# scwolof/gp_grief

Hardware: AMD Instinct MI355X
Metric: CG iters/sec + Kron-matvec achieved HBM GB/s, 4D RBF grid 200^4 (higher is better)
Workload: dtype f64

## Files before the change

### gp_grief_amd/csrc/gg_kronb.hip

```cpp
#include <algorithm>
#include <cmath>
#include <cstdlib>
#include <vector>

#include "gg_internal.h"

namespace gg {

typedef double bd4 __attribute__((ext_vector_type(4)));

constexpr int kBlkMaxD = 6;
constexpr int kBlkModeWaves = 12;
constexpr int kBlkPairWaves = 4;

struct BlockOp {
  int d = 0;
  int64_t m[kBlkMaxD] = {}, h[kBlkMaxD] = {};
  int64_t e[kBlkMaxD] = {};
  int64_t nb = 0, n = 0;
  double* frag[kBlkMaxD][2] = {};
  int KS[kBlkMaxD] = {}, JT[kBlkMaxD] = {};
  bool T4[kBlkMaxD] = {};
  int pTF = 0;
  int cus = 256;
  bool pair_lds = false;
  int pair_spw = 1;
  bool fast = true;
  bool pro_nt = true;
  bool epi_nt = true;
};

struct FoldGeom {
  int d;
  int64_t m[kBlkMaxD], h[kBlkMaxD], stride[kBlkMaxD];
  int64_t hp;
  int64_t nb;
  int64_t blk0, nblk;
};

template <int D>
__global__ __launch_bounds__(256) void blk_fold_kernel(const double* __restrict__ x,
                                                       double* __restrict__ y, FoldGeom g,
                                                       int inverse, double scale,
                                                       double* __restrict__ sq_part) {
  constexpr int C = 1 << D;
  double acc = 0.0;
  for (int64_t t = (int64_t)blockIdx.x * blockDim.x + threadIdx.x; t < g.nb;
       t += (int64_t)gridDim.x * blockDim.x) {
    int64_t lo = 0, span[D];
    const int64_t hs = g.hp;
    const int64_t q = t % (hs * hs);
    int64_t rem = t / (hs * hs);
    {
      const int64_t a4 = q / (4 * hs), r4 = q - a4 * 4 * hs;
      const int64_t i = r4 >> 2, a = 4 * a4 + (r4 & 3);
      if (i >= g.h[D - 2] || a >= g.h[D - 1]) {
        if (!inverse)
          for (int c = 0; c < C; ++c) {
            const int64_t lb = (int64_t)c - g.blk0;
            if (lb >= 0 && lb < g.nblk) y[lb * g.nb + t] = 0.0;
          }
        continue;
      }
      lo = i * g.stride[D - 2] + a * g.stride[D - 1];
      span[D - 2] = (g.m[D - 2] - 1 - 2 * i) * g.stride[D - 2];
      span[D - 1] = (g.m[D - 1] - 1 - 2 * a) * g.stride[D - 1];
    }
#pragma unroll
    for (int k = D - 3; k >= 0; --k) {
      const int64_t i = rem % g.h[k];
      rem /= g.h[k];
      lo += i * g.stride[k];
      span[k] = (g.m[k] - 1 - 2 * i) * g.stride[k];
    }
    double v[C];
    if (!inverse) {
#pragma unroll
      for (int c = 0; c < C; ++c) {
        int64_t o = lo;
#pragma unroll
        for (int k = 0; k < D; ++k)
          if ((c >> (D - 1 - k)) & 1) o += span[k];
        v[c] = x[o];
      }
    } else {
#pragma unroll
      for (int c = 0; c < C; ++c) {
        const int64_t lb = (int64_t)c - g.blk0;
        v[c] = (lb >= 0 && lb < g.nblk) ? x[lb * g.nb + t] : 0.0;
      }
    }
#pragma unroll
    for (int b = 1; b < C; b <<= 1)
#pragma unroll
      for (int c = 0; c < C; ++c)
        if (!(c & b)) {
          const double a0 = v[c], a1 = v[c | b];
          v[c] = a0 + a1;
          v[c | b] = a0 - a1;
        }
    if (!inverse) {
#pragma unroll
      for (int c = 0; c < C; ++c) {
        const int64_t lb = (int64_t)c - g.blk0;
        if (lb < 0 || lb >= g.nblk) continue;
        const double w = v[c] * scale;
        y[lb * g.nb + t] = w;
        acc = fma(w, w, acc);
      }
    } else {
#pragma unroll
      for (int c = 0; c < C; ++c) {
        int64_t o = lo;
#pragma unroll
        for (int k = 0; k < D; ++k)
          if ((c >> (D - 1 - k)) & 1) o += span[k];
        y[o] = v[c] * scale;
      }
    }
  }
  if (sq_part != nullptr) {
#pragma unroll
    for (int off = 32; off > 0; off >>= 1) acc += __shfl_xor(acc, off, 64);
    __shared__ double red[4];
    if ((threadIdx.x & 63) == 0) red[threadIdx.x >> 6] = acc;
    __syncthreads();
    if (threadIdx.x == 0) sq_part[blockIdx.x] = red[0] + red[1] + red[2] + red[3];
  }
}

__device__ __forceinline__ char* ubase(const void* p, int64_t off) {
  const uint64_t v = reinterpret_cast<uint64_t>(p) + (uint64_t)off;
  const uint32_t lo = __builtin_amdgcn_readfirstlane((uint32_t)v);
  const uint32_t hi = __builtin_amdgcn_readfirstlane((uint32_t)(v >> 32));
  uint64_t u = ((uint64_t)hi << 32) | lo;
  asm("" : "+s"(u));
  return reinterpret_cast<char*>(u);
}
__device__ __forceinline__ int64_t uni64(int64_t x) {
  const uint32_t lo = __builtin_amdgcn_readfirstlane((uint32_t)x);
  const uint32_t hi = __builtin_amdgcn_readfirstlane((uint32_t)((uint64_t)x >> 32));
  return (int64_t)(((uint64_t)hi << 32) | lo);
}
typedef __attribute__((address_space(1))) char gchar;
typedef __attribute__((address_space(1))) double gdouble;
__device__ __forceinline__ double ldu(const void* p, int64_t uoff, uint32_t voff) {
  gchar* b = reinterpret_cast<gchar*>(reinterpret_cast<uintptr_t>(ubase(p, uoff)));
  return *reinterpret_cast<const gdouble*>(b + voff);
}
__device__ __forceinline__ void stu(void* p, int64_t uoff, uint32_t voff, double v) {
  gchar* b = reinterpret_cast<gchar*>(reinterpret_cast<uintptr_t>(ubase(p, uoff)));
  *reinterpret_cast<gdouble*>(b + voff) = v;
}
template <bool NT>
__device__ __forceinline__ double lduq(const void* p, int64_t uoff, uint32_t voff) {
  if constexpr (!NT) return ldu(p, uoff, voff);
  gchar* b = reinterpret_cast<gchar*>(reinterpret_cast<uintptr_t>(ubase(p, uoff)));
  return __builtin_nontemporal_load(reinterpret_cast<const gdouble*>(b + voff));
}
template <bool NT>
__device__ __forceinline__ void stuq(void* p, int64_t uoff, uint32_t voff, double v) {
  if constexpr (!NT) {
    stu(p, uoff, voff, v);
  } else {
    gchar* b = reinterpret_cast<gchar*>(reinterpret_cast<uintptr_t>(ubase(p, uoff)));
    __builtin_nontemporal_store(v, reinterpret_cast<gdouble*>(b + voff));
  }
}
typedef double gd2v __attribute__((ext_vector_type(2)));
typedef __attribute__((address_space(1))) gd2v gd2;
__device__ __forceinline__ double2 ld2g(const double* p) {
  const gd2v v = *reinterpret_cast<const gd2*>(reinterpret_cast<uintptr_t>(p));
  return double2{v.x, v.y};
}
__device__ __forceinline__ void st2g(double* p, double2 v) {
  *reinterpret_cast<gd2*>(reinterpret_cast<uintptr_t>(p)) = gd2v{v.x, v.y};
}
struct ModeArgs {
  const double* X;
  double* Y;
  const double* fS;
  const double* fT;
  int h, KS;
  int64_t inner;
  int64_t spb;
  int64_t gpb;
  int64_t ngroups;
  int64_t per_wg;
  int64_t nb;
  int bitpos;
  int64_t blk0;
  const int* skip;
  double* r;
  const double* q_old;
  double* p_out;
  const CgScalars* sc;
  double* rr_part;
  int64_t pqo_stride;
  const double* pprev;
  const double* coef;
  double* sx;
  int64_t soff, sn, soff_h1, sn_h1, sstep;
};

template <int JT, bool T4, int KIND>
__global__ __launch_bounds__(64 * kBlkModeWaves, 1) void blk_mode_kernel(ModeArgs a) {
  constexpr int W = kBlkModeWaves;
  constexpr int TF = T4 ? JT - 1 : JT;
  constexpr int kDepth = 8;
  constexpr int NV = (KIND == 1 || KIND == 4) ? 3 : 1;
  constexpr int kSD = 2;
  extern __shared__ __attribute__((aligned(16))) double lds[];
  if (a.skip != nullptr && *a.skip) return;

  const int lane = threadIdx.x & 63;
  const int wave = __builtin_amdgcn_readfirstlane(threadIdx.x >> 6);
  const int n16 = lane & 15, kq = lane >> 4;
  const int64_t g0 = (int64_t)blockIdx.x * a.per_wg;
  const int64_t g1 = min(a.ngroups, g0 + a.per_wg);
  const int KS = a.KS;
  const int64_t cpr = a.inner >> 4;
  uint32_t o_e = (uint32_t)(((int64_t)kq * a.inner + n16) * 8);
  asm volatile("" : "+v"(o_e));
  const int64_t rstep = a.inner * 32;

  struct Cur {
    int64_t B, lg, o, cs;
  };
  auto cur_at = [&](int64_t g) {
    Cur c;
    c.B = g / a.gpb;
    c.lg = g - c.B * a.gpb;
    const int64_t ls = c.lg * W + wave;
    c.o = ls / cpr;
    c.cs = ls - c.o * cpr;
    return c;
  };
  auto cur_next = [&](Cur& c) {
    if (++c.lg == a.gpb) {
      c.lg = 0;
      ++c.B;
      c.o = 0;
      c.cs = wave;
    } else {
      c.cs += W;
      if (c.cs >= cpr) {
        c.cs -= cpr;
        ++c.o;
      }
    }
  };
  auto cur_base = [&](const Cur& c) -> int64_t {
    int64_t o = c.o, cs = c.cs;
// ... 145 lines not shown
            if (!(i < a.h)) xb = 0.0;
          }
          if (KIND == 4) {
            const bool ok = cs_valid && i < a.h;
            const double uv = i < a.h ? ring[u][1] : 0.0;
            const double yv = i < a.h ? ring[u][2] : 0.0;
            xb = fma(lz_cp, xb, fma(lz_cu, uv, lz_cy * yv));
            if (ok) {
              stu(a.p_out, (cs_base + (int64_t)4 * cs_s * a.inner) * 8, o_e, xb);
              rr_acc = fma(xb, xb, rr_acc);
            }
            if (!(i < a.h)) xb = 0.0;
          }
          const double* fs = lds + ((int64_t)cs_s * JT) * 64 + lane;
#pragma unroll
          for (int t = 0; t < TF; ++t)
            acc[t] = __builtin_amdgcn_mfma_f64_16x16x4f64(fs[t * 64], xb, acc[t], 0, 0, 0);
          if (T4) acc4 = __builtin_amdgcn_mfma_f64_4x4x4f64(fs[TF * 64], xb, acc4, 0, 0, 0);
          if (ld_n < nsteps) issue(u);
          if (KIND == 2) {
            const int64_t e = slen > 0 ? side_elem(cs_g, cs_s) : -1;
            const double2 xv = sring[u & 1][0], p0 = sring[u & 1][1], p1 = sring[u & 1][2];
            if (e >= 0) {
              double2 o;
              o.x = xv.x + (sc0 * p0.x + sc1 * p1.x);
              o.y = xv.y + (sc0 * p0.y + sc1 * p1.y);
              *reinterpret_cast<double2*>(sxo + e) = o;
            }
            side_issue(u & 1);
          }
          if (++cs_s == KS) {
            if (cs_valid) {
#pragma unroll
              for (int t = 0; t < TF; ++t)
#pragma unroll
                for (int r = 0; r < 4; ++r) {
                  if (T4 || 16 * t + 4 * r + kq < a.h)
                    stu(a.Y, (cs_base + (int64_t)(16 * t + 4 * r) * a.inner) * 8, o_e,
                        acc[t][r]);
                }
              if (T4 && 16 * TF + kq < a.h)
                stu(a.Y, (cs_base + (int64_t)16 * TF * a.inner) * 8, o_e, acc4);
            }
            zero();
            cs_s = 0;
            ++cs_g;
            cur_next(cc);
            cs_base = cur_base(cc);
            cs_valid = cur_valid(cc);
          }
        }
      }
    }
    sg0 = sg1;
  }
  if (KIND == 1 || KIND == 4) {
    __shared__ double red[2 * kBlkModeWaves];
#pragma unroll
    for (int off = 32; off > 0; off >>= 1) {
      rr_acc += __shfl_xor(rr_acc, off, 64);
      pqo_acc += __shfl_xor(pqo_acc, off, 64);
    }
    if (lane == 0) {
      red[wave] = rr_acc;
      red[W + wave] = pqo_acc;
    }
    __syncthreads();
    if (threadIdx.x == 0) {
      double s0 = 0.0, s1 = 0.0;
      for (int w = 0; w < W; ++w) {
        s0 += red[w];
        s1 += red[W + w];
      }
      if (a.rr_part != nullptr) {
        a.rr_part[blockIdx.x] = s0;
        if (a.pqo_stride > 0) a.rr_part[a.pqo_stride + blockIdx.x] = s1;
      }
    }
  }
}

__device__ __attribute__((aligned(16))) double g_blk_trash[6 * 64];

template <int KIND>
constexpr int fast_waves() {
  return KIND == 0 ? 12 : 8;
}

template <int TF, int KIND_>
__global__ __launch_bounds__(64 * fast_waves<KIND_>(), 1) void blk_mode_fast_kernel(ModeArgs a) {
  constexpr bool NT = KIND_ >= 3;
  constexpr bool RDER = KIND_ == 5;
  constexpr int KIND = (KIND_ == 3 || KIND_ == 5) ? 1 : KIND_;
  constexpr int W = fast_waves<KIND>();
  constexpr int JT = TF + 1;
  constexpr int KS = 4 * TF + 1;
  constexpr int kD = KIND == 0 ? KS : (KS % 5 == 0) ? 5 : (KS % 3 == 0) ? 3 : KS;
  extern __shared__ __attribute__((aligned(16))) double lds[];
  if (a.skip != nullptr && *a.skip) return;

  const int lane = threadIdx.x & 63;
  const int wave = __builtin_amdgcn_readfirstlane(threadIdx.x >> 6);
  const int n16 = lane & 15, kq = lane >> 4;
  const int64_t g0 = (int64_t)blockIdx.x * a.per_wg;
  const int64_t g1 = min(a.ngroups, g0 + a.per_wg);
  const int64_t cpr = a.inner >> 4;
  uint32_t o_e = (uint32_t)(((int64_t)kq * a.inner + n16) * 8);
  asm volatile("" : "+v"(o_e));
  const int64_t rstep = a.inner * 32;
  double* trash = g_blk_trash + 2 * lane;
  const uint32_t o_t = (uint32_t)(lane * 16);
  auto stq = [&](bool valid, void* p, int64_t uoff, uint32_t voff, double v) {
    void* bp = valid ? p : static_cast<void*>(g_blk_trash);
    stu(bp, valid ? uoff : 0, valid ? voff : o_t, v);
  };
  auto stq_nt = [&](bool valid, void* p, int64_t uoff, uint32_t voff, double v) {
    void* bp = valid ? p : static_cast<void*>(g_blk_trash);
    stuq<NT>(bp, valid ? uoff : 0, valid ? voff : o_t, v);
  };

  struct Cur {
    int64_t B, lg, o, cs;
  };
  auto cur_at = [&](int64_t g) {
    Cur c;
    c.B = g / a.gpb;
    c.lg = g - c.B * a.gpb;
    const int64_t ls = c.lg * W + wave;
    c.o = ls / cpr;
    c.cs = ls - c.o * cpr;
    return c;
  };
  auto cur_next = [&](Cur& c) {
    if (++c.lg == a.gpb) {
      c.lg = 0;
      ++c.B;
      c.o = 0;
      c.cs = wave;
    } else {
      c.cs += W;
      if (c.cs >= cpr) {
        c.cs -= cpr;
        ++c.o;
      }
    }
  };
  auto cur_base = [&](const Cur& c) -> int64_t {
    int64_t o = c.o, cs = c.cs;
    if (c.lg * W + wave >= a.spb) {
      o = (a.spb - 1) / cpr;
      cs = (a.spb - 1) - o * cpr;
    }
    return uni64(c.B * a.nb + o * (int64_t)a.h * a.inner + (cs << 4));
  };
  auto cur_valid = [&](const Cur& c) -> bool {
    return __builtin_amdgcn_readfirstlane((int)(c.lg * W + wave < a.spb)) != 0;
  };

  bool first = false, pqo_on = false;
  double beta = 0.0, alpha = 0.0, rr_acc = 0.0, pqo_acc = 0.0;
  if (KIND == 1) {
    first = a.sc->first != 0;
    beta = a.sc->beta;
    alpha = a.sc->pending != 0 ? a.sc->alpha : 0.0;
    pqo_on = a.pqo_stride > 0 && !first;
  }
  double lz_cy = 0.0, lz_cu = 0.0, lz_cp = 0.0;
  if (KIND == 4) {
    lz_cy = a.coef[0];
    lz_cu = a.coef[1];
    lz_cp = a.coef[2];
  }
  const bool pending = KIND == 1 && a.sc->pending != 0;
  const bool rst = !RDER || a.sc->rstored != 0;
  const double bprev = RDER ? a.sc->beta_p : 0.0;
  const double* rsrc = (KIND == 1 && !rst) ? a.pprev : a.r;
  double sc0 = 0.0, sc1 = 0.0;
  const double* sp0 = a.sx;
  const double* sp1 = a.sx;
  double* sxo = a.sx;
  int64_t slen = 0;
  if (KIND == 2) {
    const int xh = a.sc->xh;
    if (xh < 2) {
      const int64_t off = xh ? a.soff_h1 : a.soff;
      slen = xh ? a.sn_h1 : a.sn;
      sc0 = a.sc->xc[0];
      sc1 = a.sc->xc[1];
      sp0 = a.sc->xp[0] + off;
      sp1 = a.sc->xp[1] + off;
      sxo = a.sx + off;
    }
  }
  auto side_at = [&](int64_t g, int s, bool& own) -> int64_t {
    const int64_t q0 = (g * W + wave) * a.sstep;
    const int64_t e = q0 + 128 * (int64_t)s + 2 * lane;
    const int64_t hi = min(slen, q0 + a.sstep);
    own = e + 1 < hi;
    return own ? e : 0;
  };

  int64_t sg0 = g0;
  while (sg0 < g1) {
    const int64_t B0 = sg0 / a.gpb + a.blk0;
    const int par = (int)((B0 >> a.bitpos) & 1);
    const int64_t Bend = (((B0 >> a.bitpos) + 1) << a.bitpos) - a.blk0;
    const int64_t sg1 = min(g1, Bend * a.gpb);
    __syncthreads();
    {
      const double* src = par ? a.fT : a.fS;
      constexpr int nd = KS * JT * 64;
      for (int i = threadIdx.x * 2; i < nd; i += 64 * W * 2)
        *reinterpret_cast<double2*>(lds + i) = *reinterpret_cast<const double2*>(src + i);
    }
    __syncthreads();

    Cur lc = cur_at(sg0);
    int64_t lg_n = sg0;
    int64_t l_base = cur_base(lc);
    double ring[kD][3];
    double2 sring[kD][3];
    auto issue = [&](int slot, int s) {
      const int64_t ub = l_base * 8 + (int64_t)s * rstep;
      ring[slot][0] = lduq<NT>(a.X, ub, o_e);
      if (KIND == 1 || KIND == 4) {
        ring[slot][1] = lduq<NT>(KIND == 1 ? rsrc : a.r, ub, o_e);
        ring[slot][2] = lduq<NT>(a.q_old, ub, o_e);
      }
      if (KIND == 2) {
        bool own;
        const int64_t e = side_at(lg_n < sg1 ? lg_n : sg1 - 1, s, own);
        sring[slot][0] = ld2g(sxo + e);
        sring[slot][1] = ld2g(sp0 + e);
        sring[slot][2] = ld2g(sp1 + e);
      }
    };
    auto load_next_strip = [&] {
      if (lg_n + 1 < sg1) {
        cur_next(lc);
        l_base = cur_base(lc);
      }
      ++lg_n;
    };
#pragma unroll
    for (int u = 0; u < kD; ++u) issue(u, u);

    Cur cc = cur_at(sg0);
#pragma unroll 1
    for (int64_t g = sg0; g < sg1; ++g) {
      const int64_t cbase = cur_base(cc);
      const bool cvalid = cur_valid(cc);
      uint32_t lo = (uint32_t)(lane * 8);
      asm volatile("" : "+v"(lo));
      const char* lb = reinterpret_cast<const char*>(lds) + lo;
      bd4 acc[TF];
      double acc4 = 0.0;
#pragma unroll
      for (int t = 0; t < TF; ++t) acc[t] = bd4{0.0, 0.0, 0.0, 0.0};
#pragma unroll
      for (int s = 0; s < KS; ++s) {
        const int slot = s % kD;
        double xb = ring[slot][0];
        if (KIND == 1) {
          double r = rst ? ring[slot][1] : fma(-bprev, ring[slot][1], xb);
          const double q = ring[slot][2];
          const int64_t ub = (cbase + (int64_t)4 * s * a.inner) * 8;
          r = r - alpha * q;
          const double rr = fma(r, r, rr_acc);
          xb = first ? r : fma(beta, xb, r);
          const double pqo = fma(xb, q, pqo_acc);
          if (cvalid) {
            if (pending) rr_acc = rr;
            if (pqo_on) pqo_acc = pqo;
          }
          if (!RDER) stq_nt(cvalid, a.r, ub, o_e, r);
          stq_nt(cvalid, a.p_out, ub, o_e, xb);
        }
        if (KIND == 4) {
          const int64_t ub = (cbase + (int64_t)4 * s * a.inner) * 8;
          xb = fma(lz_cp, xb, fma(lz_cu, ring[slot][1], lz_cy * ring[slot][2]));
          const double rr = fma(xb, xb, rr_acc);
          if (cvalid) rr_acc = rr;
          stq_nt(cvalid, a.p_out, ub, o_e, xb);
        }
        const double* fs = reinterpret_cast<const double*>(lb + (s * JT) * 512);
#pragma unroll
        for (int t = 0; t < TF; ++t)
          acc[t] = __builtin_amdgcn_mfma_f64_16x16x4f64(fs[t * 64], xb, acc[t], 0, 0, 0);
        acc4 = __builtin_amdgcn_mfma_f64_4x4x4f64(fs[TF * 64], xb, acc4, 0, 0, 0);
        if (KIND == 2) {
          bool own;
          const int64_t e = side_at(g, s, own);
          const double2 xv = sring[slot][0], p0 = sring[slot][1], p1 = sring[slot][2];
          double2 o;
          o.x = xv.x + (sc0 * p0.x + sc1 * p1.x);
          o.y = xv.y + (sc0 * p0.y + sc1 * p1.y);
          st2g(own ? sxo + e : trash, o);
        }
// ... 687 lines not shown
    pctr = (int)((blockIdx.x / 8 + blockIdx.x / (unsigned)max(A.scus, 1)) % (unsigned)wR);
  }
  PairSlabSrc cur = src_at(0);
#pragma unroll
  for (int j = 0; j + 1 < NS; ++j) issue(cur, min(j, R::KS - 1), j);
  double pq = 0.0, qq = 0.0;
  int cslot = 0;
  for (int it = 0; it < nmine; ++it) {
    const int64_t slab = ((int64_t)blockIdx.x + (int64_t)it * G) * SPW + sl;
    const bool nv = it + 1 < nmine;
    const PairSlabSrc nxt = nv ? src_at(it + 1) : cur;
    const int role = (wave + it) & 1;
    if (role == 0)
      pair_slab_lds<TF, SPW, EPI, 0, JA, true, (SIDE & 2) != 0>(A, slab, sl, cslot, it == 0, cur, nxt, nv, ring,
                                               issue, pq, qq);
    else
      pair_slab_lds<TF, SPW, EPI, JA, TF - JA, false, (SIDE & 2) != 0>(A, slab, sl, cslot, it == 0, cur, nxt, nv,
                                                      ring, issue, pq, qq);
    if ((SIDE & 4) && slen > 0) {
      if (wR < 2) {
        side_chunk_win(((int64_t)blockIdx.x + (int64_t)it * G) * R::NW + wave);
      } else {
        pctr = pctr + 1 == wR ? 0 : pctr + 1;
        if (pctr == 0 || !nv) {
          win_phase_n(min(slen, (ufirst + pdone) * A.sstep),
                      min(slen, (ufirst + it + 1) * A.sstep));
          pdone = it + 1;
        }
      }
    } else if ((SIDE & 1) && slen > 0)
      side_chunk(((int64_t)blockIdx.x + (int64_t)it * G) * R::NW + wave);
    cslot = (cslot + R::KS) % NS;
    cur = nxt;
  }
  blk_wait_vm<0>();
  if (A.partials != nullptr) {
    __syncthreads();
    double* red = ring;
#pragma unroll
    for (int off = 32; off > 0; off >>= 1) {
      pq += __shfl_xor(pq, off, 64);
      qq += __shfl_xor(qq, off, 64);
    }
    if (lane == 0) {
      red[wave] = pq;
      red[R::NW + wave] = qq;
    }
    __syncthreads();
    if (threadIdx.x == 0) {
      double s0 = 0.0, s1 = 0.0;
      for (int w = 0; w < R::NW; ++w) {
        s0 += red[w];
        s1 += red[R::NW + w];
      }
      A.partials[blockIdx.x] = s0;
      A.partials[A.pstride + blockIdx.x] = 0.0;
      A.partials[2 * A.pstride + blockIdx.x] = s1;
    }
  }
}

typedef void (*blk_mode_fn)(ModeArgs);
typedef void (*blk_pair_fn)(PairArgs);



template <int KIND>
static blk_mode_fn mode_fn(int JT, bool T4) {
#define GG_BLK_MODE(jt)                                                    \
  case jt:                                                                 \
    return T4 ? blk_mode_kernel<jt, true, KIND> : blk_mode_kernel<jt, false, KIND>;
  switch (JT) {
    GG_BLK_MODE(1)
    GG_BLK_MODE(2)
    GG_BLK_MODE(3)
    GG_BLK_MODE(4)
    GG_BLK_MODE(5)
    GG_BLK_MODE(6)
    GG_BLK_MODE(7)
    default: return nullptr;
  }
#undef GG_BLK_MODE
}
template <int KIND>
static blk_mode_fn mode_fast_fn(int JT) {
  if (KIND != 0 && (JT == 5 || (KIND == 2 && JT == 4))) return nullptr;
  switch (JT) {
    case 2: return blk_mode_fast_kernel<1, KIND>;
    case 3: return blk_mode_fast_kernel<2, KIND>;
    case 4: return blk_mode_fast_kernel<3, KIND>;
    case 5: return blk_mode_fast_kernel<4, KIND>;
    case 6: return blk_mode_fast_kernel<5, KIND>;
    case 7: return blk_mode_fast_kernel<6, KIND>;
    default: return nullptr;
  }
}
static blk_mode_fn select_mode(int kind, int JT, bool T4, int h = 0, bool fast = false) {
  if (T4 && h == 16 * (JT - 1) + 4 && fast) {
    const blk_mode_fn f = kind == 5   ? mode_fast_fn<5>(JT)
                          : kind == 4 ? mode_fast_fn<4>(JT)
                          : kind == 3 ? mode_fast_fn<3>(JT)
                          : kind == 1 ? mode_fast_fn<1>(JT)
                          : kind == 2 ? mode_fast_fn<2>(JT)
                                      : mode_fast_fn<0>(JT);
    if (f != nullptr) return f;
  }
  return (kind == 1 || kind == 3) ? mode_fn<1>(JT, T4)
         : kind == 2              ? mode_fn<2>(JT, T4)
         : kind == 4              ? mode_fn<4>(JT, T4)
                                  : mode_fn<0>(JT, T4);
}

template <int EPI, int SIDE>
static blk_pair_fn select_pair_lds(int TF, int spw) {
  switch (TF) {
    case 2:
      return spw == 2 ? blk_pair_lds_kernel<2, 1, 2, EPI, SIDE>
                      : blk_pair_lds_kernel<2, 1, 1, EPI, SIDE>;
    case 3:
      return spw == 2 ? blk_pair_lds_kernel<3, 1, 2, EPI, SIDE>
                      : blk_pair_lds_kernel<3, 1, 1, EPI, SIDE>;
    case 4:
      return spw == 2 ? blk_pair_lds_kernel<4, 2, 2, EPI, SIDE>
                      : blk_pair_lds_kernel<4, 2, 1, EPI, SIDE>;
    case 5:
      return spw == 2 ? blk_pair_lds_kernel<5, 2, 2, EPI, SIDE>
                      : blk_pair_lds_kernel<5, 2, 1, EPI, SIDE>;
    case 6:
      return spw == 2 ? blk_pair_lds_kernel<6, 3, 2, EPI, SIDE>
                      : blk_pair_lds_kernel<6, 3, 1, EPI, SIDE>;
    default: return nullptr;
  }
}

static blk_pair_fn select_pair(int TF, bool lds = false, int spw = 1, bool epi = false,
                               bool side = false, bool nt = false, bool win = false) {
  if (lds) {
    if (side && win) return nt ? select_pair_lds<1, 7>(TF, spw) : select_pair_lds<1, 5>(TF, spw);
    if (side) return nt ? select_pair_lds<1, 3>(TF, spw) : select_pair_lds<1, 1>(TF, spw);
    if (epi && nt) return select_pair_lds<1, 2>(TF, spw);
    return epi ? select_pair_lds<1, 0>(TF, spw) : select_pair_lds<0, 0>(TF, spw);
  }
  switch (TF) {
    case 1: return blk_pair_kernel<1, 1>;
    case 2: return blk_pair_kernel<2, 1>;
    case 3: return blk_pair_kernel<3, 1>;
    case 4: return blk_pair_kernel<4, 2>;
    case 5: return blk_pair_kernel<5, 2>;
    case 6: return blk_pair_kernel<6, 3>;
    default: return nullptr;
  }
}

static int blk_cus() {
  static int n = 0;
  if (n == 0) {
    int dev = 0;
    GG_HIP(hipGetDevice(&dev));
    GG_HIP(hipDeviceGetAttribute(&n, hipDeviceAttributeMultiprocessorCount, dev));
    if (n <= 0) n = 256;
  }
  return n;
}

static void blk_set_lds_limits(const BlockOp* B) {
  for (int k = 0; k + 2 < B->d; ++k) {
    const size_t bytes = (size_t)B->KS[k] * B->JT[k] * 64 * sizeof(double);
    for (int kind = 0; kind < 6; ++kind)
      GG_HIP(hipFuncSetAttribute(
          reinterpret_cast<const void*>(
              select_mode(kind, B->JT[k], B->T4[k], (int)B->h[k], B->fast)),
          hipFuncAttributeMaxDynamicSharedMemorySize, (int)bytes));
  }
}

BlockOp* block_create(int d, const int64_t* rows, const int64_t* cols,
                      const double* const* factors) {
  if (d < 2 || d > kBlkMaxD) return nullptr;
  const char* env = gg::knob("GG_KRON_BLOCK");
  if (env && atoi(env) == 0) return nullptr;
  for (int k = 0; k < d; ++k) {
    if (rows[k] != cols[k] || rows[k] % 2 != 0 || rows[k] < 2) return nullptr;
    if (rows[k] / 2 > 112) return nullptr;
  }
  const int64_t hpair = rows[d - 1] / 2;
  if (rows[d - 2] != rows[d - 1]) return nullptr;
  const int TF = (int)std::max<int64_t>(1, ceil_div(hpair - 4, 16));
  if (select_pair(TF) == nullptr) return nullptr;
  const int64_t hp = 16 * (int64_t)TF + 4;
  for (int k = 0; k < d; ++k) {
    const int64_t m = rows[k];
    const double* F = factors[k];
    double amax = 0.0, dmax = 0.0;
    for (int64_t j = 0; j < m; ++j)
      for (int64_t i = 0; i < m; ++i) {
        amax = std::max(amax, std::fabs(F[j * m + i]));
        dmax = std::max(dmax, std::fabs(F[j * m + i] - F[(m - 1 - j) * m + (m - 1 - i)]));
      }
    if (!(dmax <= 16.0 * 2.220446049250313e-16 * amax) || !(amax > 0.0)) return nullptr;
  }
  BlockOp* B = new BlockOp();
  try {
    B->d = d;
    B->nb = 1;
    for (int k = 0; k < d; ++k) {
      B->m[k] = rows[k];
      B->h[k] = rows[k] / 2;
      B->e[k] = k >= d - 2 ? hp : B->h[k];
      B->nb *= B->e[k];
    }
    B->n = B->nb << d;
    B->pTF = TF;
    B->cus = blk_cus();
    const char* fe = gg::knob("GG_BLK_MODE_FAST");
    B->fast = !(fe && atoi(fe) == 0);
    const char* ne = gg::knob("GG_BLK_PRO_NT");
    B->pro_nt = !(ne && atoi(ne) == 0);
    const char* ee = gg::knob("GG_BLK_EPI_NT");
    B->epi_nt = !(ee && atoi(ee) == 0);
    const char* le = gg::knob("GG_BLK_PAIR_LDS");
    B->pair_lds = select_pair(TF, true) != nullptr && !(le && atoi(le) == 0);
    {
      int64_t spb = 1;
      for (int k = 0; k + 2 < d; ++k) spb *= rows[k] / 2;
      const char* se = gg::knob("GG_BLK_PAIR_SPW");
      B->pair_spw = (spb % 2 == 0 && !(se && atoi(se) == 1)) ? 2 : 1;
    }
    for (int k = 0; k < d; ++k) {
      const int64_t m = B->m[k], h = B->h[k];
      const double* F = factors[k];
      auto Fc = [&](int64_t j, int64_t i) {
        return 0.5 * (F[j * m + i] + F[(m - 1 - j) * m + (m - 1 - i)]);
      };
      int JT, KS;
      bool T4;
      if (k >= d - 2) {
        JT = TF + 1;
        T4 = true;
        KS = 4 * TF + 1;
      } else {
        const int64_t tail = h % 16;
        T4 = tail != 0 && tail <= 4;
        JT = (int)ceil_div(h, 16);
        KS = (int)ceil_div(h, 4);
      }
      B->JT[k] = JT;
      B->KS[k] = KS;
      B->T4[k] = T4;
      const int TFk = T4 ? JT - 1 : JT;
      for (int par = 0; par < 2; ++par) {
        std::vector<double> hb((size_t)KS * JT * 64 + 128, 0.0);
        for (int s = 0; s < KS; ++s)
          for (int t = 0; t < JT; ++t)
            for (int l = 0; l < 64; ++l) {
              const bool tail = T4 && t == TFk;
              const int64_t j = tail ? 16 * (int64_t)t + (l & 3) : 16 * (int64_t)t + (l & 15);
              const int64_t i = 4 * (int64_t)s + (l >> 4);
              double v = 0.0;
              if (j < h && i < h)
                v = par == 0 ? Fc(j, i) + Fc(j, m - 1 - i) : Fc(j, i) - Fc(j, m - 1 - i);
              hb[((size_t)s * JT + t) * 64 + l] = v;
            }
        GG_HIP(hipMalloc(&B->frag[k][par], hb.size() * sizeof(double)));
        GG_HIP(hipMemcpy(B->frag[k][par], hb.data(), hb.size() * sizeof(double),
                         hipMemcpyHostToDevice));
      }
    }
    for (int k = 0; k + 2 < d; ++k)
      GG_REQUIRE(select_mode(0, B->JT[k], B->T4[k]) != nullptr, GG_ERR_RUNTIME,
                 "no block mode kernel for this factor order");
    blk_set_lds_limits(B);
  } catch (...) {
    block_destroy(B);
    throw;
  }
  return B;
}

void block_destroy(BlockOp* B) {
  if (!B) return;
  for (int k = 0; k < kBlkMaxD; ++k)
    for (int p = 0; p < 2; ++p)
      if (B->frag[k][p]) (void)hipFree(B->frag[k][p]);
  delete B;
}

int64_t block_n(const BlockOp* B) { return B->n; }
int block_d(const BlockOp* B) { return B->d; }
int block_launches(const BlockOp* B) { return B->d - 1; }

static int fold_grid(const BlockOp* B) {
  return (int)std::min<int64_t>(ceil_div(B->nb, 256), (int64_t)B->cus * 8);
}
int64_t block_fold_partials(const BlockOp* B) { return fold_grid(B); }

int64_t block_nb(const BlockOp* B) { return B->nb; }

void block_fold(const BlockOp* B, bool inverse, const double* x, double* y, double* sq_part,
                hipStream_t s, int64_t blk0, int64_t nblk) {
  if (nblk < 0) {
    blk0 = 0;
    nblk = (int64_t)1 << B->d;
  }
  GG_REQUIRE(blk0 >= 0 && nblk >= 1 && blk0 + nblk <= ((int64_t)1 << B->d), GG_ERR_VALUE,
             "block range outside the 2^d blocks");
  FoldGeom g{};
  g.d = B->d;
  g.nb = B->nb;
  g.hp = B->e[B->d - 1];
  g.blk0 = blk0;
  g.nblk = nblk;
  int64_t st = 1;
  for (int k = B->d - 1; k >= 0; --k) {
    g.m[k] = B->m[k];
    g.h[k] = B->h[k];
    g.stride[k] = st;
    st *= B->m[k];
  }
  const double scale = std::ldexp(1.0, -B->d / 2) * ((B->d & 1) ? M_SQRT1_2 : 1.0);
  const int grid = fold_grid(B);
  double* sp = inverse ? nullptr : sq_part;
  switch (B->d) {
#define GG_BLK_FOLD(D)                                                                      \
  case D:                                                                                   \
    hipLaunchKernelGGL(blk_fold_kernel<D>, dim3(grid), dim3(256), 0, s, x, y, g,           \
                       inverse ? 1 : 0, scale, sp);                                         \
    break;
    GG_BLK_FOLD(2)
    GG_BLK_FOLD(3)
    GG_BLK_FOLD(4)
    GG_BLK_FOLD(5)
    GG_BLK_FOLD(6)
#undef GG_BLK_FOLD
    default: GG_REQUIRE(false, GG_ERR_VALUE, "block basis: 2 <= d <= 6");
  }
  GG_LAUNCH_CHECK();
}

static int mode_waves(int kind, const BlockOp* B, int k) {
  const int JT = B->JT[k];
  const bool fast = B->T4[k] && B->h[k] == 16 * (JT - 1) + 4 && B->fast &&
                    (kind == 5   ? mode_fast_fn<5>(JT)
                     : kind == 4 ? mode_fast_fn<4>(JT)
                     : kind == 3 ? mode_fast_fn<3>(JT)
                     : kind == 1 ? mode_fast_fn<1>(JT)
                     : kind == 2 ? mode_fast_fn<2>(JT)
                                 : mode_fast_fn<0>(JT)) != nullptr;
  if (!fast) return kBlkModeWaves;
  return kind == 0 ? fast_waves<0>() : kind == 2 ? fast_waves<2>() : fast_waves<1>();
}

static int64_t mode_geometry(const BlockOp* B, int k, int W, ModeArgs& a, int* grid_out,
                             int64_t nblk = -1) {
  const int d = B->d;
  int64_t inner = 1, outer = 1;
  for (int i = k + 1; i < d; ++i) inner *= B->e[i];
  for (int i = 0; i < k; ++i) outer *= B->h[i];
  GG_REQUIRE(inner % 16 == 0, GG_ERR_VALUE, "block basis: inner extent not a multiple of 16");
  a.h = (int)B->h[k];
  a.KS = B->KS[k];
  a.inner = inner;
  a.spb = outer * (inner / 16);
  a.gpb = ceil_div(a.spb, (int64_t)W);
  a.ngroups = a.gpb * (nblk < 0 ? ((int64_t)1 << d) : nblk);
  const int64_t grid = std::min<int64_t>(a.ngroups, (int64_t)B->cus);
  a.per_wg = ceil_div(a.ngroups, grid);
  a.nb = B->nb;
  a.bitpos = d - 1 - k;
  a.fS = B->frag[k][0];
  a.fT = B->frag[k][1];
  const int64_t g = ceil_div(a.ngroups, a.per_wg);
  *grid_out = (int)g;
  return g;
}

int64_t block_prologue_blocks(const BlockOp* B) {
  ModeArgs a{};
  int g = 0;
  if (B->d < 3) return 1;
  mode_geometry(B, 0, mode_waves(1, B, 0), a, &g);
  return g;
}

static int pair_grid(const BlockOp* B, int64_t nblk = -1) {
  const int64_t nslab = B->nb / (B->e[B->d - 1] * B->e[B->d - 2]) *
                        (nblk < 0 ? ((int64_t)1 << B->d) : nblk);
  if (B->pair_lds)
    return (int)std::min<int64_t>(nslab / B->pair_spw, (int64_t)B->cus * 4 / B->pair_spw);
  return (int)std::min<int64_t>(ceil_div(nslab, kBlkPairWaves / 2), (int64_t)B->cus * 2);
}
int64_t block_partials_needed(const BlockOp* B) { return pair_grid(B); }

void block_apply(const BlockOp* B, const double* x, double* y, double shift, double* work,
                 double* dot_partials, const int* skip, hipStream_t stream, int64_t* n_partials,
                 const MpFuse* cg, int cgp, hipEvent_t* ev, int64_t blk0, int64_t nblk) {
  const int d = B->d;
  if (nblk < 0) {
    blk0 = 0;
    nblk = (int64_t)1 << d;
  }
  GG_REQUIRE(blk0 >= 0 && nblk >= 1 && blk0 + nblk <= ((int64_t)1 << d), GG_ERR_VALUE,
             "block range outside the 2^d blocks");
  if (cg == nullptr) cgp = 0;
  GG_REQUIRE(cgp == 0 || cgp == 2 || cgp == 3, GG_ERR_VALUE,
             "block basis: plain, fused CG or fused Lanczos only");
  GG_REQUIRE(cgp == 0 || d >= 3, GG_ERR_VALUE, "block basis CG / Lanczos: d >= 3");
  GG_REQUIRE(x != y, GG_ERR_VALUE, "x and y must not alias");
  if (cgp == 2)
    GG_REQUIRE(cg->q_old == y && cg->p_out != nullptr && cg->p_out != x &&
                   cg->blk_q_out != nullptr && cg->blk_q_out != y,
               GG_ERR_VALUE, "block CG: buffer roles");
  else if (cgp == 3)
    GG_REQUIRE(cg->q_old == y && cg->p_out == x && cg->r != nullptr && cg->r != x &&
                   cg->r != y && cg->coef != nullptr && cg->blk_q_out != nullptr &&
                   cg->blk_q_out != y && cg->blk_q_out != x && cg->blk_q_out != cg->r,
               GG_ERR_VALUE, "block Lanczos: buffer roles");
  else if (d >= 3)
    GG_REQUIRE(work != nullptr && work != x && work != y, GG_ERR_VALUE,
               "block basis: scratch required");
  if (ev) GG_HIP(hipEventRecord(ev[0], stream));
  const double* src = x;
  double* chain = cgp >= 2 ? y : work;
  int pos = 0;
  const bool side = cgp == 2 && cg->sx != nullptr && (cg->xdefer == 2 || cg->xdefer == 3);
  const bool pair_side = side && B->pair_lds;
  const bool win = side && cg->xdefer == 3;
  GG_REQUIRE(!win || (pair_side && cg->xwin >= 2 && cg->xwin <= kXWinMax), GG_ERR_VALUE,
             "block CG: the x window needs the LDS pair launch");
  for (int k = 0; k + 2 < d; ++k) {
    ModeArgs a{};
    int grid = 0;
    int kind = 0;
    if (cgp == 2 && k == 0)
      kind = cg->rderive ? 5 : B->pro_nt ? 3 : 1;
    else if (cgp == 3 && k == 0)
      kind = 4;
    else if (k == 1 && side && !pair_side)
      kind = 2;
    const int W = mode_waves(kind, B, k);
    mode_geometry(B, k, W, a, &grid, nblk);
    a.blk0 = blk0;
    a.X = src;
    a.Y = chain;
    a.skip = skip;
    if (kind == 1 || kind == 3 || kind == 5) {
      a.r = cg->r;
      a.pprev = cg->pprev;
      GG_REQUIRE(kind != 5 || cg->pprev != nullptr, GG_ERR_VALUE,
                 "block CG: derived r needs p_{j-2}");
      a.q_old = cg->q_old;
      a.p_out = cg->p_out;
      a.sc = cg->sc;
      a.rr_part = cg->rr_part;
      a.pqo_stride = cg->pqo_stride;
      GG_REQUIRE(grid <= cg->rr_cap, GG_ERR_VALUE, "prologue partial array too short");
      if (cg->pro_blocks != nullptr) *cg->pro_blocks = grid;
    } else if (kind == 4) {
      a.r = cg->r;
      a.q_old = cg->q_old;
      a.p_out = cg->p_out;
      a.coef = cg->coef;
      a.rr_part = cg->rr_part;
      GG_REQUIRE(grid <= cg->rr_cap, GG_ERR_VALUE, "prologue partial array too short");
      if (cg->pro_blocks != nullptr) *cg->pro_blocks = grid;
    } else if (kind == 2) {
      a.sc = cg->sc;
      a.sx = cg->sx;
      const int64_t sn = cg->sn;
      const int64_t H = block_side_half(sn);
      a.soff = 0;
      a.sn = std::min(H, sn);
      a.soff_h1 = a.sn;
      a.sn_h1 = sn - a.sn;
      const int64_t slots = a.ngroups * W;
      a.sstep = 2 * ceil_div(std::max<int64_t>(std::max(a.sn, a.sn_h1), 1), 2 * slots);
      GG_REQUIRE(a.sstep <= 128 * (int64_t)a.KS, GG_ERR_VALUE,
                 "block CG: x side job larger than its k-steps");
    }
    const blk_mode_fn fn = select_mode(kind, B->JT[k], B->T4[k], (int)B->h[k], B->fast);
    const size_t lds = (size_t)B->KS[k] * B->JT[k] * 64 * sizeof(double);
    hipLaunchKernelGGL(fn, dim3(grid), dim3(64 * W), lds, stream, a);
    GG_LAUNCH_CHECK();
    if (k == 0 && d == 3 && side && !pair_side)
      launch_x_half(cg->sx, cg->sn, block_side_half(cg->sn), cg->sc, stream);
    if (ev) GG_HIP(hipEventRecord(ev[++pos], stream));
    src = chain;
  }
  PairArgs p{};
  p.X = src;
  p.Y = cgp >= 2 ? cg->blk_q_out : y;
  const int k3 = d - 1, k2 = d - 2;
  p.f3S = B->frag[k3][0];
  p.f3T = B->frag[k3][1];
  p.f2S = B->frag[k2][0];
  p.f2T = B->frag[k2][1];
  p.spb = B->nb / (B->e[k3] * B->e[k2]);
  p.nslab = p.spb * nblk;
  p.blk0 = blk0;
  p.skip = skip;
  const int grid = pair_grid(B, nblk);
  if (cgp >= 2) {
    p.P = cg->p_out;
    p.shift = shift;
    p.partials = dot_partials;
    p.pstride = cg->pstride;
  } else if (shift != 0.0) {
    p.P = x;
    p.shift = shift;
  }
  if (pair_side && win) {
    p.sc = cg->sc;
    p.sx = cg->sx;
    p.sn = cg->sn;
    p.sreg_len = xwin_region(cg->sn, cg->xwin);
    GG_REQUIRE(cg->sn % 2 == 0, GG_ERR_VALUE, "block CG: the x window takes x in pairs");
    p.sphase = cg->xphase >= 1 && cg->xphase <= kXWinPhaseMax ? cg->xphase : kXWinPhaseDefault;
    p.scus = B->cus;
    const int64_t units = p.nslab / B->pair_spw;
    if (p.sphase >= 2) {
      p.sstep = 16 * ceil_div(std::max<int64_t>(p.sreg_len, 1), 16 * units);
    } else {
      const int64_t slots = units * 2 * B->pair_spw;
      p.sstep = 2 * ceil_div(std::max<int64_t>(p.sreg_len, 1), 2 * slots);
    }
  } else if (pair_side) {
    p.sc = cg->sc;
    p.sx = cg->sx;
    const int64_t sn = cg->sn;
    const int64_t H = block_side_half(sn);
    p.soff = 0;
    p.sn = std::min(H, sn);
    p.soff_h1 = p.sn;
    p.sn_h1 = sn - p.sn;
    const int64_t slots = p.nslab / B->pair_spw * 2 * B->pair_spw;
    p.sstep = 2 * ceil_div(std::max<int64_t>(std::max(p.sn, p.sn_h1), 1), 2 * slots);
  }
  hipLaunchKernelGGL(select_pair(B->pTF, B->pair_lds, B->pair_spw, p.P != nullptr, pair_side,
                                 B->epi_nt && (pair_side || cgp == 3), win),
                     dim3(grid), dim3(B->pair_lds ? 128 * B->pair_spw : 64 * kBlkPairWaves), 0,
                     stream, p);
  GG_LAUNCH_CHECK();
  if (ev) GG_HIP(hipEventRecord(ev[++pos], stream));
  if (n_partials) *n_partials = (cgp >= 2) ? grid : 0;
}

int64_t block_side_half(int64_t n) { return 2 * ceil_div(n, (int64_t)4); }

bool block_pair_side(const BlockOp* B) { return B != nullptr && B->pair_lds; }

bool block_rderive_ok(const BlockOp* B) {
  if (B == nullptr || B->d < 3 || !B->pro_nt) return false;
  const int JT = B->JT[0];
  return B->T4[0] && B->h[0] == 16 * (JT - 1) + 4 && B->fast && mode_fast_fn<5>(JT) != nullptr;
}

bool block_efficient(const BlockOp* B) {
  if (B == nullptr) return false;
  const int d = B->d;
  return B->e[d - 1] == B->h[d - 1] && B->e[d - 2] == B->h[d - 2];
}

}
// ... 1 lines not shown
```

Measured before the change: 32.01.

## Process two column strips per wave in block mode kernels with 16-byte accesses

Adds a two-strip variant of the fast block mode-product kernel. Each lane now loads and stores pairs of doubles as 16-byte vectors, and each LDS factor fragment is reused across two MFMA accumulator sets. This is enabled by default for the plain and CG-prologue kinds. The goal is to halve LDS factor reads per output and widen global memory transactions. In exchange it uses more registers per wave, drops kind 0 from 12 to 8 waves, and adds handling for an odd strip count through half-strip offsets and trash stores.

```diff
diff --git a/gp_grief_amd/csrc/gg_kronb.hip b/gp_grief_amd/csrc/gg_kronb.hip
--- a/gp_grief_amd/csrc/gg_kronb.hip
+++ b/gp_grief_amd/csrc/gg_kronb.hip
@@ -12,6 +12,7 @@
 constexpr int kBlkMaxD = 6;
 constexpr int kBlkModeWaves = 12;
 constexpr int kBlkPairWaves = 4;
+constexpr int kBlkModeStripsDefault = 3;
 
 struct BlockOp {
   int d = 0;
@@ -26,6 +27,7 @@
   bool pair_lds = false;
   int pair_spw = 1;
   bool fast = true;
+  int strips = kBlkModeStripsDefault;
   bool pro_nt = true;
   bool epi_nt = true;
 };
@@ -169,6 +171,22 @@
 }
 typedef double gd2v __attribute__((ext_vector_type(2)));
 typedef __attribute__((address_space(1))) gd2v gd2;
+template <bool NT>
+__device__ __forceinline__ gd2v lduq2(const void* p, int64_t uoff, uint32_t voff) {
+  gchar* b = reinterpret_cast<gchar*>(reinterpret_cast<uintptr_t>(ubase(p, uoff)));
+  if constexpr (!NT) return *reinterpret_cast<const gd2*>(b + voff);
+  return __builtin_nontemporal_load(reinterpret_cast<const gd2*>(b + voff));
+}
+template <bool NT>
+__device__ __forceinline__ void stw2(bool own, void* p, int64_t uoff, uint32_t voff, gchar* tp,
+                                     gd2v v) {
+  gchar* b = reinterpret_cast<gchar*>(reinterpret_cast<uintptr_t>(ubase(p, uoff)));
+  gd2* q = reinterpret_cast<gd2*>(own ? b + voff : tp);
+  if constexpr (!NT)
+    *q = v;
+  else
+    __builtin_nontemporal_store(v, q);
+}
 __device__ __forceinline__ double2 ld2g(const double* p) {
   const gd2v v = *reinterpret_cast<const gd2*>(reinterpret_cast<uintptr_t>(p));
   return double2{v.x, v.y};
@@ -480,17 +498,20 @@
 
 __device__ __attribute__((aligned(16))) double g_blk_trash[6 * 64];
 
-template <int KIND>
+template <int KIND, int SW = 1>
 constexpr int fast_waves() {
-  return KIND == 0 ? 12 : 8;
-}
-
-template <int TF, int KIND_>
-__global__ __launch_bounds__(64 * fast_waves<KIND_>(), 1) void blk_mode_fast_kernel(ModeArgs a) {
+  return (KIND == 0 && SW == 1) ? 12 : 8;
+}
+
+template <int TF, int KIND_, int SW = 1>
+__global__ __launch_bounds__((64 * fast_waves<KIND_, SW>()), 1) void blk_mode_fast_kernel(ModeArgs a) {
+  static_assert(SW == 1 || SW == 2, "one or two strips per wave");
+  static_assert(SW == 1 || (KIND_ != 2 && KIND_ != 4),
+                "the side-job and Lanczos kinds stay at one strip per wave");
   constexpr bool NT = KIND_ >= 3;
   constexpr bool RDER = KIND_ == 5;
   constexpr int KIND = (KIND_ == 3 || KIND_ == 5) ? 1 : KIND_;
-  constexpr int W = fast_waves<KIND>();
+  constexpr int W = fast_waves<KIND, SW>();
   constexpr int JT = TF + 1;
   constexpr int KS = 4 * TF + 1;
   constexpr int kD = KIND == 0 ? KS : (KS % 5 == 0) ? 5 : (KS % 3 == 0) ? 3 : KS;
@@ -502,9 +523,17 @@
   const int n16 = lane & 15, kq = lane >> 4;
   const int64_t g0 = (int64_t)blockIdx.x * a.per_wg;
   const int64_t g1 = min(a.ngroups, g0 + a.per_wg);
-  const int64_t cpr = a.inner >> 4;
-  uint32_t o_e = (uint32_t)(((int64_t)kq * a.inner + n16) * 8);
+  const int64_t cpr = ((a.inner >> 4) + (SW - 1)) / SW;
+  const bool odd = SW == 2 && ((a.inner >> 4) & 1) != 0;
+  uint32_t o_e = (uint32_t)(((int64_t)kq * a.inner + SW * n16) * 8);
   asm volatile("" : "+v"(o_e));
+  [[maybe_unused]] uint32_t o_h = 0;
+  [[maybe_unused]] bool lo8 = true;
+  if constexpr (SW == 2) {
+    o_h = (uint32_t)(((int64_t)kq * a.inner + 2 * (n16 & 7)) * 8);
+    asm volatile("" : "+v"(o_h));
+    lo8 = n16 < 8;
+  }
   const int64_t rstep = a.inner * 32;
   double* trash = g_blk_trash + 2 * lane;
   const uint32_t o_t = (uint32_t)(lane * 16);
@@ -516,6 +545,9 @@
     void* bp = valid ? p : static_cast<void*>(g_blk_trash);
     stuq<NT>(bp, valid ? uoff : 0, valid ? voff : o_t, v);
   };
+  [[maybe_unused]] gchar* tp2 = nullptr;
+  if constexpr (SW == 2)
+    tp2 = reinterpret_cast<gchar*>(reinterpret_cast<uintptr_t>(g_blk_trash)) + o_t;
 
   struct Cur {
     int64_t B, lg, o, cs;
@@ -549,10 +581,15 @@
       o = (a.spb - 1) / cpr;
       cs = (a.spb - 1) - o * cpr;
     }
-    return uni64(c.B * a.nb + o * (int64_t)a.h * a.inner + (cs << 4));
+    return uni64(c.B * a.nb + o * (int64_t)a.h * a.inner + cs * (16 * SW));
   };
   auto cur_valid = [&](const Cur& c) -> bool {
     return __builtin_amdgcn_readfirstlane((int)(c.lg * W + wave < a.spb)) != 0;
+  };
+  auto cur_half = [&](const Cur& c) -> bool {
+    if (SW == 1) return false;
+    const bool last = c.lg * W + wave >= a.spb || c.cs == cpr - 1;
+    return __builtin_amdgcn_readfirstlane((int)(odd && last)) != 0;
   };
 
   bool first = false, pqo_on = false;
@@ -612,6 +649,103 @@
         *reinterpret_cast<double2*>(lds + i) = *reinterpret_cast<const double2*>(src + i);
     }
     __syncthreads();
+
+    if constexpr (SW == 2) {
+      Cur lc = cur_at(sg0);
+      int64_t lg_n = sg0;
+      int64_t l_base = cur_base(lc);
+      uint32_t l_oe = cur_half(lc) ? o_h : o_e;
+      gd2v ring[kD][3];
+      auto issue = [&](int slot, int s) {
+        const int64_t ub = l_base * 8 + (int64_t)s * rstep;
+        ring[slot][0] = lduq2<NT>(a.X, ub, l_oe);
+        if (KIND == 1) {
+          ring[slot][1] = lduq2<NT>(rsrc, ub, l_oe);
+          ring[slot][2] = lduq2<NT>(a.q_old, ub, l_oe);
+        }
+      };
+      auto load_next_strip = [&] {
+        if (lg_n + 1 < sg1) {
+          cur_next(lc);
+          l_base = cur_base(lc);
+          l_oe = cur_half(lc) ? o_h : o_e;
+        }
+        ++lg_n;
+      };
+#pragma unroll
+      for (int u = 0; u < kD; ++u) issue(u, u);
+
+      Cur cc = cur_at(sg0);
+#pragma unroll 1
+      for (int64_t g = sg0; g < sg1; ++g) {
+        const int64_t cbase = cur_base(cc);
+        const bool chalf = cur_half(cc);
+        const uint32_t c_oe = chalf ? o_h : o_e;
+        const bool own = cur_valid(cc) && (lo8 || !chalf);
+        const bool own_rr = own && pending, own_pq = own && pqo_on;
+        uint32_t lo = (uint32_t)(lane * 8);
+        asm volatile("" : "+v"(lo));
+        const char* lb = reinterpret_cast<const char*>(lds) + lo;
+        bd4 acc[2][TF];
+        double acc4[2] = {0.0, 0.0};
+#pragma unroll
+        for (int t = 0; t < TF; ++t) acc[0][t] = acc[1][t] = bd4{0.0, 0.0, 0.0, 0.0};
+#pragma unroll
+        for (int s = 0; s < KS; ++s) {
+          const int slot = s % kD;
+          gd2v xb = ring[slot][0];
+          if (KIND == 1) {
+            const gd2v q = ring[slot][2];
+            const int64_t ub = (cbase + (int64_t)4 * s * a.inner) * 8;
+            gd2v r;
+#pragma unroll
+            for (int c = 0; c < 2; ++c) {
+              double rc = rst ? ring[slot][1][c] : fma(-bprev, ring[slot][1][c], xb[c]);
+              rc = rc - alpha * q[c];
+              const double rr = fma(rc, rc, rr_acc);
+              xb[c] = first ? rc : fma(beta, xb[c], rc);
+              const double pqo = fma(xb[c], q[c], pqo_acc);
+              rr_acc = own_rr ? rr : rr_acc;
+              pqo_acc = own_pq ? pqo : pqo_acc;
+              r[c] = rc;
+            }
+            if (!RDER) stw2<NT>(own, a.r, ub, c_oe, tp2, r);
+            stw2<NT>(own, a.p_out, ub, c_oe, tp2, xb);
+          }
+          const double* fs = reinterpret_cast<const double*>(lb + (s * JT) * 512);
+#pragma unroll
+          for (int t = 0; t < TF; ++t) {
+            const double f = fs[t * 64];
+            acc[0][t] = __builtin_amdgcn_mfma_f64_16x16x4f64(f, xb.x, acc[0][t], 0, 0, 0);
+            acc[1][t] = __builtin_amdgcn_mfma_f64_16x16x4f64(f, xb.y, acc[1][t], 0, 0, 0);
+          }
+          {
+            const double f = fs[TF * 64];
+            acc4[0] = __builtin_amdgcn_mfma_f64_4x4x4f64(f, xb.x, acc4[0], 0, 0, 0);
+            acc4[1] = __builtin_amdgcn_mfma_f64_4x4x4f64(f, xb.y, acc4[1], 0, 0, 0);
+          }
+          if (s + kD < KS) {
+            issue(slot, s + kD);
+          } else {
+            if (s + kD == KS) load_next_strip();
+            issue(slot, s + kD - KS);
+          }
+          if (KIND == 1) asm volatile("" : "+v"(rr_acc), "+v"(pqo_acc));
+          __builtin_amdgcn_sched_barrier(0);
+        }
+#pragma unroll
+        for (int t = 0; t < TF; ++t)
+#pragma unroll
+          for (int r = 0; r < 4; ++r)
+            stw2<false>(own, a.Y, (cbase + (int64_t)(16 * t + 4 * r) * a.inner) * 8, c_oe, tp2,
+                        gd2v{acc[0][t][r], acc[1][t][r]});
+        stw2<false>(own, a.Y, (cbase + (int64_t)16 * TF * a.inner) * 8, c_oe, tp2,
+                    gd2v{acc4[0], acc4[1]});
+        cur_next(cc);
+      }
+      sg0 = sg1;
+      continue;
+    }
 
     Cur lc = cur_at(sg0);
     int64_t lg_n = sg0;
@@ -1465,28 +1599,39 @@
   }
 #undef GG_BLK_MODE
 }
-template <int KIND>
+template <int KIND, int SW = 1>
 static blk_mode_fn mode_fast_fn(int JT) {
   if (KIND != 0 && (JT == 5 || (KIND == 2 && JT == 4))) return nullptr;
   switch (JT) {
-    case 2: return blk_mode_fast_kernel<1, KIND>;
-    case 3: return blk_mode_fast_kernel<2, KIND>;
-    case 4: return blk_mode_fast_kernel<3, KIND>;
-    case 5: return blk_mode_fast_kernel<4, KIND>;
-    case 6: return blk_mode_fast_kernel<5, KIND>;
-    case 7: return blk_mode_fast_kernel<6, KIND>;
+    case 2: return blk_mode_fast_kernel<1, KIND, SW>;
+    case 3: return blk_mode_fast_kernel<2, KIND, SW>;
+    case 4: return blk_mode_fast_kernel<3, KIND, SW>;
+    case 5: return blk_mode_fast_kernel<4, KIND, SW>;
+    case 6: return blk_mode_fast_kernel<5, KIND, SW>;
+    case 7: return blk_mode_fast_kernel<6, KIND, SW>;
     default: return nullptr;
   }
 }
-static blk_mode_fn select_mode(int kind, int JT, bool T4, int h = 0, bool fast = false) {
+static blk_mode_fn mode_fast_of(int kind, int JT, int sw) {
+  if (sw == 2)
+    return kind == 5   ? mode_fast_fn<5, 2>(JT)
+           : kind == 3 ? mode_fast_fn<3, 2>(JT)
+           : kind == 1 ? mode_fast_fn<1, 2>(JT)
+           : kind == 0 ? mode_fast_fn<0, 2>(JT)
+                       : nullptr;
+  return kind == 5   ? mode_fast_fn<5>(JT)
+         : kind == 4 ? mode_fast_fn<4>(JT)
+         : kind == 3 ? mode_fast_fn<3>(JT)
+         : kind == 1 ? mode_fast_fn<1>(JT)
+         : kind == 2 ? mode_fast_fn<2>(JT)
+                     : mode_fast_fn<0>(JT);
+}
+static blk_mode_fn select_mode(int kind, int JT, bool T4, int h = 0, bool fast = false,
+                               int sw = 1) {
   if (T4 && h == 16 * (JT - 1) + 4 && fast) {
-    const blk_mode_fn f = kind == 5   ? mode_fast_fn<5>(JT)
-                          : kind == 4 ? mode_fast_fn<4>(JT)
-                          : kind == 3 ? mode_fast_fn<3>(JT)
-                          : kind == 1 ? mode_fast_fn<1>(JT)
-                          : kind == 2 ? mode_fast_fn<2>(JT)
-                                      : mode_fast_fn<0>(JT);
+    const blk_mode_fn f = mode_fast_of(kind, JT, sw);
     if (f != nullptr) return f;
+    GG_REQUIRE(sw == 1, GG_ERR_RUNTIME, "no two-strip block mode kernel for this launch");
   }
   return (kind == 1 || kind == 3) ? mode_fn<1>(JT, T4)
          : kind == 2              ? mode_fn<2>(JT, T4)
@@ -1546,13 +1691,21 @@
   return n;
 }
 
+static int mode_sw(int kind, const BlockOp* B, int k) {
+  const int JT = B->JT[k];
+  if (!(B->T4[k] && B->h[k] == 16 * (JT - 1) + 4 && B->fast)) return 1;
+  const int bit = kind == 0 ? 1 : (kind == 1 || kind == 3 || kind == 5) ? 2 : 0;
+  if ((B->strips & bit) == 0) return 1;
+  return mode_fast_of(kind, JT, 2) != nullptr ? 2 : 1;
+}
+
 static void blk_set_lds_limits(const BlockOp* B) {
   for (int k = 0; k + 2 < B->d; ++k) {
     const size_t bytes = (size_t)B->KS[k] * B->JT[k] * 64 * sizeof(double);
     for (int kind = 0; kind < 6; ++kind)
       GG_HIP(hipFuncSetAttribute(
-          reinterpret_cast<const void*>(
-              select_mode(kind, B->JT[k], B->T4[k], (int)B->h[k], B->fast)),
+          reinterpret_cast<const void*>(select_mode(kind, B->JT[k], B->T4[k], (int)B->h[k],
+                                                    B->fast, mode_sw(kind, B, k))),
           hipFuncAttributeMaxDynamicSharedMemorySize, (int)bytes));
   }
 }
@@ -1597,6 +1750,8 @@
     B->cus = blk_cus();
     const char* fe = gg::knob("GG_BLK_MODE_FAST");
     B->fast = !(fe && atoi(fe) == 0);
+    const char* st = gg::knob("GG_BLK_MODE_STRIPS");
+    if (st) B->strips = atoi(st) & 3;
     const char* ne = gg::knob("GG_BLK_PRO_NT");
     B->pro_nt = !(ne && atoi(ne) == 0);
     const char* ee = gg::knob("GG_BLK_EPI_NT");
@@ -1723,18 +1878,14 @@
 static int mode_waves(int kind, const BlockOp* B, int k) {
   const int JT = B->JT[k];
   const bool fast = B->T4[k] && B->h[k] == 16 * (JT - 1) + 4 && B->fast &&
-                    (kind == 5   ? mode_fast_fn<5>(JT)
-                     : kind == 4 ? mode_fast_fn<4>(JT)
-                     : kind == 3 ? mode_fast_fn<3>(JT)
-                     : kind == 1 ? mode_fast_fn<1>(JT)
-                     : kind == 2 ? mode_fast_fn<2>(JT)
-                                 : mode_fast_fn<0>(JT)) != nullptr;
+                    mode_fast_of(kind, JT, 1) != nullptr;
   if (!fast) return kBlkModeWaves;
+  if (kind == 0 && mode_sw(kind, B, k) == 2) return fast_waves<0, 2>();
   return kind == 0 ? fast_waves<0>() : kind == 2 ? fast_waves<2>() : fast_waves<1>();
 }
 
 static int64_t mode_geometry(const BlockOp* B, int k, int W, ModeArgs& a, int* grid_out,
-                             int64_t nblk = -1) {
+                             int64_t nblk = -1, int sw = 1) {
   const int d = B->d;
   int64_t inner = 1, outer = 1;
   for (int i = k + 1; i < d; ++i) inner *= B->e[i];
@@ -1743,7 +1894,7 @@
   a.h = (int)B->h[k];
   a.KS = B->KS[k];
   a.inner = inner;
-  a.spb = outer * (inner / 16);
+  a.spb = outer * ceil_div(inner / 16, (int64_t)sw);
   a.gpb = ceil_div(a.spb, (int64_t)W);
   a.ngroups = a.gpb * (nblk < 0 ? ((int64_t)1 << d) : nblk);
   const int64_t grid = std::min<int64_t>(a.ngroups, (int64_t)B->cus);
@@ -1762,7 +1913,7 @@
   int g = 0;
   if (B->d < 3) return 1;
   mode_geometry(B, 0, mode_waves(1, B, 0), a, &g);
-  return g;
+  return std::min<int64_t>(a.ngroups, (int64_t)B->cus);
 }
 
 static int pair_grid(const BlockOp* B, int64_t nblk = -1) {
@@ -1821,7 +1972,8 @@
     else if (k == 1 && side && !pair_side)
       kind = 2;
     const int W = mode_waves(kind, B, k);
-    mode_geometry(B, k, W, a, &grid, nblk);
+    const int sw = mode_sw(kind, B, k);
+    mode_geometry(B, k, W, a, &grid, nblk, sw);
     a.blk0 = blk0;
     a.X = src;
     a.Y = chain;
@@ -1860,7 +2012,8 @@
       GG_REQUIRE(a.sstep <= 128 * (int64_t)a.KS, GG_ERR_VALUE,
                  "block CG: x side job larger than its k-steps");
     }
-    const blk_mode_fn fn = select_mode(kind, B->JT[k], B->T4[k], (int)B->h[k], B->fast);
+    const blk_mode_fn fn =
+        select_mode(kind, B->JT[k], B->T4[k], (int)B->h[k], B->fast, sw);
     const size_t lds = (size_t)B->KS[k] * B->JT[k] * 64 * sizeof(double);
     hipLaunchKernelGGL(fn, dim3(grid), dim3(64 * W), lds, stream, a);
     GG_LAUNCH_CHECK();
```

Measured after the change: 32.65, median of 6. +2.0%, better.
